# DataCanvasIO/DeepTables

Hardware: AMD Instinct MI355X
Metric: training rows/sec (fwd+bwd) DeepFM Criteo-shape batch 8192 (higher is better)
Workload: dtype f32 (split-bf16: 24-bit fwd / 16-bit bwd)

## Files before the change

### deeptables_amd/_lib.py

```python
import ctypes
import os

import torch

_HERE = os.path.dirname(os.path.abspath(__file__))
LIB_PATH = os.path.join(_HERE, 'libdt_hip.so')

_c_int = ctypes.c_int
_c_i64 = ctypes.c_int64
_c_f32 = ctypes.c_float
_ptr = ctypes.c_void_p

SIGNATURES = {
    'dt_version': (_c_int, []),
    'dt_last_error': (ctypes.c_char_p, []),
    'dt_build_arch': (ctypes.c_char_p, []),
    'dt_source_hash': (ctypes.c_char_p, []),
    'dt_graph_upload': (_c_int, [_ptr, _ptr]),
    'dt_step_trace': (_c_int, [_c_int]),
    'dt_step_trace_read': (_c_int, [_ptr, _c_int, _ptr]),
    'dt_embedding_fwd': (_c_int, [_ptr, _c_int, _ptr, _ptr, _ptr, _c_int, _c_int, _c_int, _ptr, _ptr,
                                  _ptr, _ptr]),
    'dt_embedding_bwd_dense': (_c_int, [_ptr, _ptr, _c_int, _c_int, _ptr, _ptr]),
    'dt_fm_fwd': (_c_int, [_ptr, _c_int, _c_int, _c_int, _ptr, _ptr]),
# ... 92 lines not shown
    'dt_deepfm_train_step': (_c_int, [_ptr, _c_int, _ptr, _ptr, _ptr, _ptr, _ptr, _c_int, _c_int, _c_int, _c_int,
                                      _ptr, _ptr, _ptr, _ptr, _ptr, _c_f32, _c_f32, _ptr, _ptr, _ptr, _ptr, _ptr,
                                      _ptr, _ptr, _ptr, _ptr, _ptr, _ptr, _ptr, _ptr, _ptr, _c_i64, _c_f32, _c_int, _c_int,
                                      _c_f32, _ptr, _c_f32, _ptr, _ptr]),
    'dt_deepfm_train_step_adam': (_c_int, [_ptr, _c_int, _ptr, _ptr, _ptr, _ptr, _ptr, _c_int, _c_int, _c_int, _c_int,
                                           _ptr, _ptr, _ptr, _ptr, _ptr, _c_f32, _c_f32, _ptr, _ptr, _ptr, _ptr, _ptr,
                                           _ptr, _ptr, _ptr, _ptr, _ptr, _ptr, _ptr, _ptr, _ptr, _c_i64, _c_int,
                                           _c_f32, _ptr, _c_f32, _ptr, _ptr, _ptr, _c_int, _ptr, _c_f32, _c_f32, _c_f32, _c_f32,
                                           _ptr, _ptr, _ptr, _c_i64, _c_f32, _ptr, _ptr, _ptr, _ptr]),
    'dt_deepfm_step_chains': (_c_int, [_c_int] * 5),
    'dt_deepfm_dropout_hash': (ctypes.c_uint32, [ctypes.c_uint32] * 3),
    'dt_feed_gather': (_c_int, [_ptr, _c_i64, _c_int, _ptr, _ptr, _ptr, _ptr, _ptr]),
    'dt_embedding_gather_owned': (_c_int, [_ptr, _c_int, _ptr, _ptr, _ptr, _c_int, _c_int, _c_int, _c_int, _c_int,
                                           _c_int, _ptr, _ptr, _ptr, _ptr]),
    'dt_deepfm_preelect': (_c_int, [_ptr, _c_int, _ptr, _ptr, _c_int, _c_int, _ptr, _ptr, _c_i64, _ptr]),
    'dt_deepfm_dedupe_slots': (_c_i64, [_c_int, _c_int]),
    'dt_deepfm_dedupe_bytes': (_c_i64, [_c_int, _c_int]),
    'dt_deepfm_dedupe_segments': (_c_int, [_c_int, _c_int, _ptr]),
    'dt_deepfm_dedupe_overflow_offset': (_c_i64, [_c_int, _c_int]),
    'dt_dcn_supported': (_c_int, [_c_int] * 7),
    'dt_dcn_workspace_bytes': (_c_i64, [_c_int] * 5),
    'dt_dcn_stamps_offset_floats': (_c_i64, [_c_int] * 5),
    'dt_dcn_accum_floats': (_c_i64, [_c_int] * 4),
    'dt_dcn_accum_offsets': (_c_int, [_c_int, _c_int, _c_int, _c_int, _ptr]),
    'dt_dcn_train_step': (_c_int, [_ptr, _c_int, _ptr, _ptr, _ptr, _ptr, _ptr, _c_int, _c_int, _c_int, _c_int,
                                   _ptr, _ptr, _c_int, _ptr, _ptr, _ptr, _ptr, _c_f32, _c_f32,
                                   _ptr, _ptr, _ptr, _ptr, _ptr, _ptr, _ptr,
                                   _ptr, _ptr, _ptr, _ptr, _ptr, _ptr, _ptr, _c_i64, _c_int, _c_f32, _ptr, _c_f32, _ptr, _ptr]),
    'dt_dcn_train_step_adam': (_c_int, [_ptr, _c_int, _ptr, _ptr, _ptr, _ptr, _ptr, _c_int, _c_int, _c_int, _c_int,
                                        _ptr, _ptr, _c_int, _ptr, _ptr, _ptr, _ptr, _c_f32, _c_f32,
# ... 38 lines not shown
    'dt_xdeepfm_infer_cin': (_c_int, [_c_int, _ptr, _ptr, _ptr, _c_int, _c_int, _c_int, _c_int, _c_int, _c_int, _ptr, _c_int,
                                      _c_int, _ptr, _ptr, _ptr]),
    'dt_xdeepfm_infer_head': (_c_int, [_ptr, _ptr, _c_int, _c_int, _c_int, _c_int, _c_int, _ptr, _c_int, _c_int, _ptr, _ptr,
                                       _ptr, _c_int, _ptr]),
}

DT_IDX_F32, DT_IDX_I32 = 0, 1
DT_AI_F32, DT_AI_BF16, DT_AI_BF16X2 = 0, 1, 2
DT_STEP_LOSS_MSE = 0x10
DT_STEP_SKIP_FINISH, DT_STEP_FINISH_ONLY = 0x20, 0x40
DT_STEP_TOWER_X3 = 0x80
DT_STEP_PREELECTED = 0x100
DT_STEP_TOWER_BF16 = 0x200
DT_STEP_STAMPS = 0x400
DT_STEP_PREPARED = 0x800
DT_INFER_SIGMOID, DT_INFER_TOWER_BF16 = 0x1, 0x2
DT_NET_LINEAR, DT_NET_FM, DT_NET_DNN = 0x1, 0x2, 0x4
DT_CIN_F32, DT_CIN_BF16, DT_CIN_BF16X3 = 0, 1, 2
DT_XDEEPFM_MAX_LAYERS = 8
DT_FEED_CURSOR_WORDS = 528
DT_ACT_LINEAR, DT_ACT_RELU = 0, 1
ACT_CODES = {None: 0, 'linear': 0, 'relu': 1, 'sigmoid': 2, 'tanh': 3, 'elu': 4, 'selu': 5, 'softplus': 6, 'softsign': 7,
             'exponential': 8}


def act_code(name, what):
    if name not in ACT_CODES:
        raise ValueError(f'{what} activation {name!r}: the HIP kernels fuse {sorted(k for k in ACT_CODES if k)}')
    return ACT_CODES[name]
DT_OP_KERNEL = {'mat': 0, 'vec': 1, 'num': 2}
# ... 46 lines not shown
```

### deeptables_amd/compiled.py

```python
import ctypes
import os

import torch

from . import _lib, training
from ._lib import check, lib, ptr, stream_ptr


def _hip_graph_upload(graph):
    try:
        handle = graph.raw_cuda_graph_exec()
    except (AttributeError, RuntimeError):
        return False
    return lib().dt_graph_upload(ctypes.c_void_p(int(handle)), stream_ptr()) == 0


class _old_garbage_frozen:

    def __enter__(self):
        import gc
        self.app_frozen = gc.get_freeze_count() > 0
        gc.collect()
        if not self.app_frozen:
            gc.freeze()
# ... 40 lines not shown
        self.opt_graph = None
        self._dp_steps = 0
        self._opt_graph_sig = None
        self._last_exchange_sig = None
        self._opt_graph_refused = False
        self._sig_objects = None
        self._sparse_refs = None
        self.logits = None
        self.losses = None
        self._out_refs, self._graph_out_refs, self._outputs_by_ref = {}, None, False
        self.phase_events = None
        self._first_events = None
        self._slots_per_step = False
        self.preelected = False
        self.chained = False
        self.uploaded = False
        srcs = list(feed.blocks) + ([] if self.slot_y is None else [feed.y])
        dsts = list(self.slots) + ([] if self.slot_y is None else [self.slot_y])
        nb = len(srcs)
        if nb > 8 or any((t.element_size() * (t.numel() // max(t.shape[0], 1))) % 4 for t in srcs):
            self._gather_args = False
        else:
            arr = ctypes.c_void_p * nb
            self._gather_args = (arr(*[t.data_ptr() for t in srcs]), arr(*[t.data_ptr() for t in dsts]),
                                 (ctypes.c_int * nb)(*[t.element_size() * (t.numel() // t.shape[0]) for t in srcs]), nb)

    @staticmethod
    def _nccl_backend(st):
        try:
            import torch.distributed as dist
# ... 64 lines not shown
    def steps_left(self):
        return (self.rows_available() - self.pos) // self.B

    def _gather(self, steps=None):
        n = (self.k if steps is None else steps) * self.B
        if self._gather_args is False:
            for blk, slot in zip(self.feed.blocks, self.slots):
                torch.index_select(blk, 0, self.sel[:n], out=slot[:n])
            if self.slot_y is not None:
                torch.index_select(self.feed.y, 0, self.sel[:n], out=self.slot_y[:n])
            return
        src, dst, rb, nb = self._gather_args
        check(lib().dt_feed_gather(ptr(self.order_buf), n, nb, ctypes.cast(src, ctypes.c_void_p),
                                   ctypes.cast(dst, ctypes.c_void_p), ctypes.cast(rb, ctypes.c_void_p), ptr(self.cursor),
                                   stream_ptr()), 'dt_feed_gather')

    def _step_inputs(self, i):
        s, e = i * self.B, (i + 1) * self.B
        ins = [sl[s:e] for sl in self.slots]
        yb = None if self.slot_y is None else self.slot_y[s:e]
        wb = None
        if self.feed.weighted:
            wb, yb = yb[:, -1].contiguous(), yb[:, :-1].contiguous()
            if self.feed.y_ndim == 1:
                yb = yb.reshape(-1)
        return ins, yb, wb

    def _sharded(self):
        st = self.strategy
        return self.dp and getattr(st, 'sharded_embeddings', False) and st.active and self.dm.fused_plan() is not None

    @staticmethod
    def _id_slot(i, chained):
        if not chained or i == 0:
            return i
        return 1 + ((i - 1) & 1)

    def _body(self, i, core_only=False, preelected=False, chained=False):
        dm = self.dm
        ins, yb, wb = self._step_inputs(i)
        if core_only:
            plan = dm.fused_plan()
            dm.optimizer.zero_grad(flat=False)
            loss, logit = plan.sharded_core(self.B, ins[1] if len(ins) > 1 else None, yb, self.strategy, wb)
            dm.model._dt_flat_grad = plan.accum
            return
        fused_opt = self.with_optimizer and not self.dp
        chain = {}
        if chained:
            if i + 1 < self.k:
                chain['next_ids'] = (self.slots[0][(i + 1) * self.B:(i + 2) * self.B], self._id_slot(i + 1, True))
            chain['prepared'] = i >= 1
        loss, logit = dm._forward_backward(ins, yb, wb, apply_rows=fused_opt and self.strategy is None,
                                           logit_out=None if self.logits is None else self.logits[i],
                                           slot=self._id_slot(i, chained) if self._slots_per_step else 0,
                                           preelected=preelected, **chain)
        if fused_opt:
            dm.optimizer.step()
        used_plan = getattr(dm, '_step_used_plan', False)
        if self.logits is None:
            self.logits = torch.empty((self.k,) + tuple(logit.shape), dtype=logit.dtype, device=logit.device)
            self.losses = torch.zeros(self.k, dtype=torch.float32, device=logit.device)
        self._outputs_by_ref = not used_plan and not self.dp
        if self._outputs_by_ref:
            self._out_refs[i] = (loss.detach().reshape(()), logit.detach())
        else:
            if logit.data_ptr() != self.logits[i].data_ptr():
                self.logits[i].copy_(logit)
            if not used_plan:
                self.losses[i].copy_(loss.reshape(()))
        self._losses_from_logits = bool(used_plan)

    def capture(self, warm_steps=2, collect=None):
        dm = self.dm
        dm.model.train()
        s = torch.cuda.Stream()
        s.wait_stream(torch.cuda.current_stream())
        with torch.cuda.stream(s):
            for _ in range(warm_steps):
                self._eager_steps(1, collect)
        torch.cuda.current_stream().wait_stream(s)
        torch.cuda.synchronize()
        if self._dp_graph_wanted:
            g = self._capture_dp_whole()
            if self.strategy.world_size > 1:
                import torch.distributed as dist
# ... 3 lines not shown
                    g = None
            if g is not None:
                self.graph, self.dp_graph = g, True
                import weakref
                self._owner = tuple(None if o is None else weakref.ref(o)
                                    for o in (dm.model, dm.optimizer, getattr(dm, '_fused_plan', None)))
                self.uploaded = _hip_graph_upload(g)
                torch.cuda.synchronize()
                return warm_steps
            self.k = 1
        if not self.use_graph or (self._sharded() and not self.graph_segments):
            return warm_steps
        from .models.layers import MultiColumnEmbedding
        emb_layers = [l for l in dm.model.modules() if isinstance(l, MultiColumnEmbedding)]
        core_only = self._sharded()
        plan = dm.fused_plan()
        pre = (self.k > 1 and not self.dp and not core_only and plan is not None and plan.can_preelect(self.B) and
               self.feed.kinds[0] == 'cat' and self.slots[0].dtype in (torch.int32, torch.float32))
        chain = (not pre and self.k > 1 and not self.dp and not core_only and self.with_optimizer and plan is not None and
                 plan.can_chain(self.B) and self.feed.kinds[0] == 'cat' and
                 self.slots[0].dtype in (torch.int32, torch.float32) and not self.feed.weighted)
        self.chained = bool(chain)
        self._slots_per_step = bool(pre or chain)
        self.preelected = bool(pre)
        if pre or chain:
            for i in range(1, self.k):
                plan._slot_buffers(self.B, self._id_slot(i, chain))
        g = torch.cuda.CUDAGraph()
        with _old_garbage_frozen():
            with torch.cuda.graph(g):
                if not core_only:
                    self._gather()
                if pre:
                    main = torch.cuda.current_stream()
                    side = torch.cuda.Stream()
                    side.wait_stream(main)
                    with torch.cuda.stream(side):
                        for i in range(1, self.k):
                            plan.preelect(self.slots[0][i * self.B:(i + 1) * self.B], slot=i)
                for i in range(self.k):
                    if pre and i == 1:
                        torch.cuda.current_stream().wait_stream(side)
                    self._body(i, core_only=core_only, preelected=pre and i >= 1, chained=chain)
        self._slots_per_step = False
        self._graph_out_refs = dict(self._out_refs) if self._outputs_by_ref else None
        self.graph = g
        import weakref
        self._owner = tuple(None if o is None else weakref.ref(o)
                            for o in (dm.model, dm.optimizer, getattr(dm, '_fused_plan', None)))
        self._sparse_refs = [(l, {key: list(v) for key, v in l.sparse_grads.items()}) for l in emb_layers]
        for layer in emb_layers:
            if not self.dp and self.with_optimizer:
                layer.sparse_grads.clear()
        torch.cuda.synchronize()
        self.uploaded = _hip_graph_upload(g)
        torch.cuda.synchronize()
        return warm_steps

# ... 193 lines not shown
```

### deeptables_amd/csrc/deepfm.hip

```cpp
#include <stdlib.h>
#include "tile_common.h"
#include "tower_x3.h"
#include "adam_dev.h"

namespace dt {

typedef float floatx4_t __attribute__((ext_vector_type(4)));

struct DeepFmAccum {
    int64_t dW1, dW2, db1, db2, dw3, dwo, dbo, loss, dgamma, dbeta, dwlin, slin, total;
    int64_t dw3d, dcw, dcb, sumc, sumcx;
};
__host__ __device__ inline DeepFmAccum deepfm_accum_layout(int C, int CP, int F, int Nd, int L = 0) {
    DeepFmAccum a;
    int64_t o = 0;
    a.dW1 = o; o += (int64_t)C * kH1;
    a.dW2 = o; o += (int64_t)kH1 * kH2;
    a.db1 = o; o += kH1;
    a.db2 = o; o += kH2;
    a.dw3 = o; o += (L > 0 ? C : 0);
    a.dw3d = o; o += kH2;
    a.dwo = o; o += 1;
    a.dbo = o; o += 1;
    a.loss = o; o += 2;
// ... 464 lines not shown
                }
            }
        }
    }
}
constexpr size_t kElectLds = (size_t)kElectSlots * 8 + kElectSlots / 32 * sizeof(unsigned) + 16 * sizeof(int);
constexpr size_t kElectLdsBig = kElectLds + (size_t)kElectList * sizeof(int);

__global__ __launch_bounds__(1024) void k_elect(DedupeWs dd, DeepFmDims dm, int64_t* __restrict__ rows_out) {
    extern __shared__ unsigned long long eslots_dyn[];
    ElectSync sy{nullptr, 0u};
    if (dd.seg_cur)
        elect_block_big<1024, false>(eslots_dyn, dd, dm.B, dm.F, (int)blockIdx.x, (int)threadIdx.x, rows_out, sy);
    else
        elect_block<1024, false>(eslots_dyn, dd, dm.B, dm.F, (int)blockIdx.x, (int)threadIdx.x, rows_out, sy);
}

template <int KIND>
__global__ __launch_bounds__(256) void k_rows_of_ids(const void* __restrict__ idx, const int64_t* __restrict__ row_offset,
                                                     const int32_t* __restrict__ vocab, DeepFmDims dm,
                                                     int64_t* __restrict__ rows_out, int64_t* __restrict__ rows_fm,
                                                     int* __restrict__ seg_cur, int* __restrict__ list_cur,
                                                     unsigned char* __restrict__ pid_fm, int pid_stride, int parts_log2) {
    __shared__ int64_t tile[64][129];
    if (blockIdx.x == 0 && seg_cur && (int)threadIdx.x < ((dm.F + 7) & ~7)) { seg_cur[threadIdx.x] = 0; list_cur[threadIdx.x] = 0; }
    const int b0 = blockIdx.x * 64;
    const int nb = min(64, dm.B - b0);
    for (int e = threadIdx.x; e < nb * dm.F; e += blockDim.x) {
        const int r = e / dm.F, f = e - r * dm.F;
        const int id = load_id<KIND>(idx, (int64_t)(b0 + r) * dm.F + f);
// ... 1649 lines not shown
    const DedupeLayout dl = dedupe_layout(B, F);
    const DedupeWs dd = dedupe_view(dedupe_ws, dl);
    DeepFmDims dm{B, F, 0, 0, 0, 0};
    if (idx_kind == DT_IDX_F32)
        hipLaunchKernelGGL(k_rows_of_ids<DT_IDX_F32>, dim3(ceil_div(B, 64)), dim3(256), 0, st, idx, row_offset, vocab, dm, rows_out,
                           dd.rows_fm, dd.seg_cur, dd.list_cur, dd.pid_fm, dd.pid_stride, dd.parts_log2);
    else
        hipLaunchKernelGGL(k_rows_of_ids<DT_IDX_I32>, dim3(ceil_div(B, 64)), dim3(256), 0, st, idx, row_offset, vocab, dm, rows_out,
                           dd.rows_fm, dd.seg_cur, dd.list_cur, dd.pid_fm, dd.pid_stride, dd.parts_log2);
    const size_t ldsB = dl.by_field ? kElectLdsBig : kElectLds;
    hipFuncSetAttribute((const void*)k_elect, hipFuncAttributeMaxDynamicSharedMemorySize, (int)ldsB);
    hipLaunchKernelGGL(k_elect, dim3(dl.eblocks), dim3(1024), ldsB, st, dd, dm, rows_out);
    return launch_status("dt_deepfm_preelect");
}

struct StepDense {
    float *p, *m, *v;
    int64_t n_flat;
    void* state;
    float lr;
};

struct StepChain {
    const void* next_idx;
    int64_t* next_rows_out;
    void* next_dedupe_ws;
};
static bool step_chains(const DeepFmDims& dm, int phases, bool with_dense, bool with_dedupe) {
    const bool x3_flag = (phases & (DT_STEP_TOWER_X3 | DT_STEP_TOWER_BF16)) != 0;
    return (phases & 0xf) == 2 && !(phases & (DT_STEP_SKIP_FINISH | DT_STEP_FINISH_ONLY)) && x3_flag && dm.CP <= 512 &&
// ... 85 lines not shown
    DT_REQUIRE(idx && table && row_offset && vocab && y && (dcn || w_lin) && bn_gamma && bn_beta && W1 && b1 && W2 && b2 &&
                   w3 && w_out && logit_out && rows_out && grad_rows && accum && workspace,
               "dt_deepfm_train_step: null pointer");
    DT_REQUIRE(Nd == 0 || dense, "dt_deepfm_train_step: dense is null");
    DT_REQUIRE(idx_kind == DT_IDX_F32 || idx_kind == DT_IDX_I32, "dt_deepfm_train_step: idx_kind %d", idx_kind);
    hipStream_t st = as_stream(stream);
    const DeepFmWs wl = deepfm_ws_layout(dm, Lc);
    const DeepFmAccum al = deepfm_accum_layout(dm.C, dm.CP, F, Nd, Lc);
    float* ws = reinterpret_cast<float*>(workspace);
    const int mse = (phases & DT_STEP_LOSS_MSE) ? 1 : 0;
    const bool skip_finish = (phases & DT_STEP_SKIP_FINISH) != 0, finish_only = (phases & DT_STEP_FINISH_ONLY) != 0;
    const bool bf16_flag = (phases & DT_STEP_TOWER_BF16) != 0;
    const bool x3_flag = (phases & DT_STEP_TOWER_X3) != 0 || bf16_flag;
    const bool prepared = (phases & DT_STEP_PREPARED) != 0;
    const bool preelected = (phases & DT_STEP_PREELECTED) != 0 || prepared;
    const int phases_all = phases;
    const bool stamps_flag = (phases & DT_STEP_STAMPS) != 0;
    phases &= 0xf;
    DT_REQUIRE(!(skip_finish && finish_only), "dt_deepfm_train_step: DT_STEP_SKIP_FINISH and DT_STEP_FINISH_ONLY together");
    const DcnArgs dca{cross_w, cross_b, w3, Lc, ws + wl.dXc, mse, 0, sample_weight, ws + wl.gpart, (Lc + 1) * dm.CP};
    const GPart gpt{dcn ? ws + wl.gpart : nullptr, (Lc + 1) * dm.CP, ceil_div(B, kTM), ws + wl.gsum};
    MlpParams mp{b1, W2, b2, dcn ? w3 + dm.C : w3, w_out, b_out, bn_gamma, ws + wl.mean, ws + wl.rstd, ws + wl.sc, ws + wl.betap,
                 W1, ws + wl.W1L, ws + wl.W2L, ws + wl.W2TL,
                 reinterpret_cast<const double*>(ws + wl.bnacc), bn_beta, bn_eps, bn_momentum, bn_moving_mean, bn_moving_var,
                 ws + wl.mean, ws + wl.rstd, ws + wl.sc, ws + wl.betap, ws + wl.gammap};
    DT_REQUIRE(((uintptr_t)W1 | (uintptr_t)W2 | (uintptr_t)(dcn ? W2 : w3) | (uintptr_t)accum) % 16 == 0,
               "dt_deepfm_train_step: W1 / W2 / w3 / accum must be 16-byte aligned");
    const int tiles = ceil_div(B, kTM);
    DedupeWs dd{nullptr, 0, nullptr, nullptr, nullptr, nullptr, nullptr};
    DT_REQUIRE(!(dedupe_ws && grad_rows_field_major), "dt_deepfm_train_step: dedupe and field-major row gradients "
// ... 46 lines not shown
        const int rec_blocks_f = ceil_div(part3_layout(dm.CP, Lc, 1).n, 256);
        const RecSrc rsrc_f{reinterpret_cast<const double*>(ws + wl.racc), part3_layout(dm.CP, Lc, 1).stride};
        hipLaunchKernelGGL(k_bn_grads2, dim3(dm.C + kH2 + rec_blocks_f), dim3(256), 0, st, W1, bn_gamma, bn_beta, dm,
                           accum, al, ws + wl.wpart, wgrad_row_blocks(), Lc, cross_w, cross_b, w3, rsrc_f, dm.C + kH2, gpt);
        if (drop.thr || drop.thr_dense) hipLaunchKernelGGL(k_emb_drop_advance, dim3(1), dim3(1), 0, st, dropout_seed);
        return launch_status(dcn ? "dt_dcn_train_step" : "dt_deepfm_train_step");
    }
    DT_REQUIRE(!adam || (pipe && dd.rows_fm && !grad_rows_field_major),
               "dt_deepfm_train_step_adam: the in-step row update needs a backward step with the in-step dedupe (dedupe_ws) "
               "and row-major row gradients");

    const bool chains = step_chains(dm, phases_all, adam && sdense, dd.rows_fm != nullptr);
    DT_REQUIRE(!prepared || chains, "dt_deepfm_train_step: DT_STEP_PREPARED on a step that cannot be chained (dt_deepfm_step_chains)");
    DT_REQUIRE(!(chain && chain->next_idx) || (chains && chain->next_rows_out && chain->next_dedupe_ws),
               "dt_deepfm_train_step_adam: next_idx on a step that cannot be chained, or without next_rows_out / next_dedupe_ws");
    StepNext nx{nullptr, nullptr, dd, 0};
    if (chain && chain->next_idx) {
        DT_REQUIRE((uintptr_t)chain->next_dedupe_ws % 16 == 0 && chain->next_dedupe_ws != dedupe_ws && chain->next_rows_out != rows_out,
                   "dt_deepfm_train_step_adam: the next step needs its own rows_out / dedupe_ws (16-byte aligned)");
        const DedupeLayout dln = dedupe_layout(B, F);
        nx.idx = chain->next_idx;
        nx.rows_out = chain->next_rows_out;
        nx.dd = dedupe_view(chain->next_dedupe_ws, dln);
        nx.eblocks = dln.eblocks;
    }
    const size_t ldsC = ((size_t)kTM * (dm.CP + kPad) + 4 * dm.CP + kTM * (kH1 + kPad) + kTM * kH2S + 5 * kTM +
                         (dcn ? kCrossLds + (2 * Lc + 1) * dm.CP : 0)) * sizeof(float);
    DT_UNSUPPORTED(ldsC > 160 * 1024, "dt_dcn_train_step: the tile kernel needs %zu B of LDS", ldsC);
    if (adam && sdense) {
        const int64_t want_flat = dcn ? al.dcb + (int64_t)Lc * dm.C : al.dwlin + F + Nd;
// ... 104 lines not shown
                           stamps ? stamps + (int64_t)tiles * 32 : nullptr, ep, ad, drop,                                 \
                           stamps ? stamps + (int64_t)tiles * 16 : nullptr, join_env, bnacc, (int)wl.bnacc_n, nx, gpt,    \
                           (adam && sdense) ? ws + wl.lrsnap : nullptr);                                               \
    } while (0)
        if (dcn) { if (wm == 0) DT_ED(true, 0); else if (wm == 1) DT_ED(true, 1); else DT_ED(true, 2); }
        else { if (wm == 0) DT_ED(false, 0); else if (wm == 1) DT_ED(false, 1); else DT_ED(false, 2); }
#undef DT_ED
        trace_mark(3, st);
        if (adam && sdense) {
            const int seg_blocks = 1024;
            const int small_blocks = rec_blocks;
            const DedupeLayout dl = dedupe_layout(B, F);
            const FinishSeg fs{SegTail{dd.nseg, dd.seg_row, dd.seg_off, dd.seg_cnt, dd.seg_list, dl.regions, dl.cap},
                               adam->table, adam->m, adam->v, grad_rows, adam->sstride, D};
            const DenseAdam da{sdense->p, sdense->m, sdense->v, adam->lr_t_host, adam->b1, adam->b2, adam->eps};
            const X3Lay lay = nx.idx ? X3Lay{x3_w1b, x3_w1r, x3_w2b, x3_w2r, n1, n1, n2, n2, dcn ? x3_cwp : nullptr}
                                     : X3Lay{nullptr, nullptr, nullptr, nullptr, 0, 0, 0, 0, nullptr};
            hipLaunchKernelGGL(k_finish_step, dim3(dm.C + kH2 + small_blocks + seg_blocks), dim3(256), 0, st, W1, ws + wl.gammap,
                               ws + wl.betap, dm, accum, al, ws + wl.wpart, row_blocks, da, (AdamState*)sdense->state, sdense->lr,
                               dm.C + kH2, small_blocks, seg_blocks, fs, Lc, cross_w, cross_b, w3, rsrc, lay, gpt, ws + wl.lrsnap);
            trace_mark(4, st);
        } else if (!skip_finish) {
            hipLaunchKernelGGL(k_bn_grads2, dim3(dm.C + kH2 + rec_blocks), dim3(256), 0, st, W1, bn_gamma, bn_beta, dm,
                               accum, al, ws + wl.wpart, row_blocks, Lc, cross_w, cross_b, w3, rsrc, dm.C + kH2, gpt);
        }
        if ((drop.thr || drop.thr_dense) && !skip_finish)
            hipLaunchKernelGGL(k_emb_drop_advance, dim3(1), dim3(1), 0, st, dropout_seed);
    } else {
        hipLaunchKernelGGL(k_finish_records, dim3(max(rec_blocks, 8)), dim3(256), 0, st, dm, accum, al, Lc, rsrc, bnacc,
                           (int)wl.bnacc_n);
    }
// ... 148 lines not shown
```

### deeptables_amd/fused.py

```python
import ctypes
import os

import torch

from . import _lib
from ._lib import check, lib, ptr, stream_ptr
from .ops import SparseRowGrad
from .utils import consts

def _step_loss(dm):
    ln = getattr(dm, 'loss_name', None)
    if dm.task == consts.TASK_BINARY and ln == 'binary_crossentropy':
        return 0
    if dm.task == consts.TASK_REGRESSION and ln in ('mse', 'mean_squared_error'):
        return _lib.DT_STEP_LOSS_MSE
    return None


TILE_H1, TILE_H2 = 128, 64


def _tower_widths(dnn_params):
    hu = tuple(tuple(h) for h in dnn_params.get('hidden_units', ()))
    if len(hu) != 2 or any(len(h) != 3 for h in hu):
# ... 236 lines not shown
    def can_preelect(self, B):
        st = self.dm.config.distribute_strategy
        return bool(st is None and _dedupe_in_step(self, B, True) and os.environ.get('DT_AMD_PREELECT', '0') == '1')

    def preelect(self, idx, slot):
        B = idx.shape[0]
        sb = self._slot_buffers(B, slot)
        idx = idx.contiguous()
        kind = _lib.DT_IDX_F32 if idx.dtype == torch.float32 else _lib.DT_IDX_I32
        if idx.dtype not in (torch.float32, torch.int32):
            raise ValueError('preelect: ids must be float32 or int32')
        check(lib().dt_deepfm_preelect(ptr(idx), kind, ptr(getattr(self.emb, f'row_offset_{self.key}')),
                                       ptr(getattr(self.emb, f'vocab_{self.key}')), B, self.F, ptr(sb['rows']),
                                       ptr(sb['dedupe']), sb['dedupe_slots'], stream_ptr()), 'dt_deepfm_preelect')

    def _phases(self, backward=True, part=0, pre=0, diag=True):
        phases = (2 if backward else 1) | part | _step_loss(self.dm) | pre
        if backward and part != _lib.DT_STEP_FINISH_ONLY:
            phases |= self.tower_flag | (self.diag_flag if diag else 0)
        return phases

    def _head(self, ids, kind, rows_src, dense, y, B, logit, rows, buf, oob, dedupe, dedupe_slots):
        training, bn = self.dm.model.training, self.bn
        return (ptr(ids), kind, *[ptr(t) for t in rows_src], ptr(dense), ptr(y), B, self.F, self.D, self.Nd,
                *self._net_args(), ptr(bn.gamma), ptr(bn.beta), ptr(bn.moving_mean) if training else None,
                ptr(bn.moving_variance) if training else None, float(bn.epsilon), float(bn.momentum), ptr(self.d1.kernel),
                ptr(self.d1.bias), ptr(self.d2.kernel), ptr(self.d2.bias), *self._head_weights(), ptr(self.out.bias),
                ptr(logit), ptr(rows), ptr(buf['grad_rows']), ptr(self.accum), ptr(buf['ws']), oob, dedupe, dedupe_slots)

    def _tail(self, phases, sw):
# ... 80 lines not shown
    def _whole_in_step(self, opt):
        table = self.emb.tables[self.key]
        flat = getattr(opt, '_flat', None)
        return bool(flat is not None and flat[0] is self.flat_params and flat[1] is self.accum and
                    os.environ.get('DT_AMD_STEP_IN_STEP', '1') != '0' and
                    all(id(p) in flat[5] for p in opt.params if p is not table))

    def can_chain(self, B):
        if os.environ.get('DT_AMD_CHAIN', '1') == '0' or self.dm.config.distribute_strategy is not None:
            return False
        opt = _rows_in_step(self, B, True, True) if _dedupe_in_step(self, B, True) else None
        if opt is None or not self._whole_in_step(opt):
            return False
        return bool(lib().dt_deepfm_step_chains(B, self.F, self.D, self.Nd, self._phases(diag=False)))

    def _id_buffers(self, idx, backward, dedupe, opt, slot, preelected, next_ids, prepared):
        B = idx.shape[0]
        ids = self._slot_buffers(B, slot) if (slot and dedupe) else self._buffers(B)
        pre = _lib.DT_STEP_PREELECTED if (preelected and dedupe and backward) else 0
        if preelected and not pre:
            raise _lib.DtHipError('a pre-elected step needs the in-step dedupe (backward, single process)')
        nxt = (None, None, None)
        if prepared or next_ids is not None:
            if opt is None or not dedupe:
                raise _lib.DtHipError('chained steps need the in-step dedupe and optimizer (can_chain)')
            if prepared:
                pre |= _lib.DT_STEP_PREPARED
            if next_ids is not None:
                nidx, nslot = next_ids
                if nidx.dtype != idx.dtype or nidx.shape != idx.shape or not nidx.is_contiguous() or not nslot or nslot == slot:
                    raise ValueError('next_ids: (contiguous ids like this step\'s, a slot of their own)')
                nb = self._slot_buffers(B, nslot)
                nxt = (ptr(nidx), ptr(nb['rows']), ptr(nb['dedupe']))
        return ids, pre, nxt

    def run(self, idx, dense, y, backward=True, apply_rows=False, sample_weight=None, logit_out=None, slot=0,
            preelected=False, next_ids=None, prepared=False):
        st = self.dm.config.distribute_strategy
        if self.ROW_OWNED and backward and getattr(st, 'sharded_embeddings', False) and st.active and \
                not self.emb.uses_dense_grad(self.D):
            return self._run_sharded(idx, dense, y, st, sample_weight)
        self.dm.model._dt_sharded_step = False
        B = idx.shape[0]
        buf = self._buffers(B)
        idx = idx.contiguous()
        kind = _lib.DT_IDX_F32 if idx.dtype == torch.float32 else _lib.DT_IDX_I32
        if idx.dtype not in (torch.float32, torch.int32):
            idx = idx.to(torch.int32)
        dense = None if dense is None else dense.contiguous()
        y = y.reshape(-1).contiguous()
        sw = _row_weights(sample_weight, y)
        table = self.emb.tables[self.key]
        logit = buf['logit']
        if logit_out is not None:
            if logit_out.shape != logit.shape or logit_out.dtype != logit.dtype or not logit_out.is_contiguous():
                raise ValueError(f'logit_out must be a contiguous float32 {tuple(logit.shape)} tensor')
            logit = logit_out
        dedupe = _dedupe_in_step(self, B, backward)
        opt = _rows_in_step(self, B, backward, apply_rows)
        ids, pre, nxt = self._id_buffers(idx, backward, dedupe, opt, slot, preelected, next_ids, prepared)
        head = self._head(idx, kind, (table, getattr(self.emb, f'row_offset_{self.key}'),
                                      getattr(self.emb, f'vocab_{self.key}')), dense, y, B, logit, ids['rows'], buf,
                          ptr(self.emb.oob_count) if self.emb.check_oob else None,
                          ptr(ids['dedupe']) if dedupe else None, buf['dedupe_slots'])
        if opt is not None:
            slots = opt._st(table, rows=True)
            whole = self._whole_in_step(opt)
            flat = opt._flat
            dn = (ptr(flat[0]), ptr(flat[2]), ptr(flat[3]), int(flat[4]), float(opt.lr)) if whole else (None, None, None, 0, 0.0)
            check(self._entry('train_step_adam')(
                *head, *self._tail(self._phases(pre=pre), sw), ptr(slots['m']), ptr(slots['v']), int(slots['m'].stride(0)),
                ptr(opt._state_tensor(table.device)), 0.0, opt.b1, opt.b2, opt.eps, *dn, *nxt, stream_ptr()),
                f'dt_{self.PREFIX}_train_step_adam')
            if whole:
                opt.applied_in_step()
# ... 437 lines not shown
```

### deeptables_amd/models/deepmodel.py

```python
import collections
import math
import os
import pickle
from collections import OrderedDict
from typing import Union

import numpy as np
import torch

from . import deepnets
from .layers import MultiColumnEmbedding, VarLenColumnEmbedding, dt_custom_objects
from .. import functional as F
from .. import training
from ..functional import Dense, Concatenate, Flatten, Input, Add, BatchNormalization, Dropout, Model
from ..utils import consts


def default_device():
    if not torch.cuda.is_available():
        raise RuntimeError('deeptables_amd needs a ROCm GPU (MI355X): the layers hot path has no CPU fallback.')
    return torch.device('cuda', torch.cuda.current_device())


class DeepModel:
# ... 217 lines not shown
            self._fused_plan = make_fused_plan(self)
        return self._fused_plan

    def inference_plan(self):
        from ..fused import make_inference_plan, predict_enabled
        if not predict_enabled() or self.model is None:
            return None
        if not hasattr(self, '_inference_plan'):
            self._inference_plan = make_inference_plan(self)
        return self._inference_plan

    def forward_backward(self, inputs, y, sample_weight=None, logit_out=None):
        return self._forward_backward(inputs, y, sample_weight, logit_out=logit_out)

    def _forward_backward(self, inputs, y, sample_weight=None, apply_rows=False, logit_out=None, slot=0, preelected=False,
                          next_ids=None, prepared=False):
        plan = self.fused_plan() if self.model.training else None
        if plan is not None and sample_weight is not None and not getattr(plan, 'takes_sample_weight', False):
            plan = None
        self.optimizer.zero_grad(flat=plan is None) if hasattr(self.optimizer, 'register_flat_group') \
            else self.optimizer.zero_grad()
        self._step_used_plan = plan is not None
        if plan is not None:
            cat = inputs[0]
            dense = inputs[1] if len(inputs) > 1 else None
            loss, logit = plan.run(cat, dense, y, apply_rows=apply_rows, sample_weight=sample_weight, logit_out=logit_out,
                                   slot=slot, preelected=preelected, next_ids=next_ids, prepared=prepared)
            self.model._dt_flat_grad = plan.accum
            return loss[0], logit
        self.model._dt_flat_grad = getattr(self, '_generic_flat_grad', None)
        self.model._dt_sharded_step = False
        logit = self.model(inputs)
        loss = self._loss(logit, y) if sample_weight is None else \
            training.weighted_loss(self.loss_name, logit, y, sample_weight)
        if loss.dim() == 0 and loss.dtype == torch.float32:
            loss.backward(training.unit_grad(loss.device))
        else:
            loss.backward()
        return loss.detach(), logit.detach()

    def train_step(self, inputs, y, sample_weight=None):
        strategy = self.config.distribute_strategy
# ... 341 lines not shown
```

### include/dt_hip.h

```cpp
#ifndef DT_HIP_H
#define DT_HIP_H

#include <stdint.h>

#ifdef __cplusplus
extern "C" {
#endif

#define DT_OK 0
#define DT_ERR_INVALID_ARG (-1)
#define DT_ERR_UNSUPPORTED (-2)
#define DT_ERR_LAUNCH (-3)

#define DT_IDX_F32 0
#define DT_IDX_I32 1

#define DT_ACT_LINEAR 0
#define DT_ACT_RELU 1
#define DT_ACT_SIGMOID 2
#define DT_ACT_TANH 3
#define DT_ACT_ELU 4
#define DT_ACT_SELU 5
#define DT_ACT_SOFTPLUS 6
#define DT_ACT_SOFTSIGN 7
// ... 196 lines not shown
int dt_field_pool_fwd(const float* x, int B, int F, int D, int use_max, float* z, int* argmax, void* stream);
int dt_field_pool_bwd(const float* grad_z, const int* argmax, int B, int F, int D, int use_max, float* grad_x,
                      void* stream);
int dt_field_scale_fwd(const float* x, const float* a, int B, int F, int D, float* out, void* stream);
int dt_field_scale_bwd(const float* x, const float* a, const float* grad_out, int B, int F, int D, float* grad_x,
                       float* grad_a, void* stream);

#define DT_STEP_LOSS_MSE 0x10
#define DT_STEP_SKIP_FINISH 0x20
#define DT_STEP_FINISH_ONLY 0x40
#define DT_STEP_TOWER_X3 0x80
#define DT_STEP_PREELECTED 0x100
#define DT_STEP_TOWER_BF16 0x200
#define DT_STEP_STAMPS 0x400
#define DT_STEP_PREPARED 0x800
int dt_deepfm_step_chains(int B, int F, int D, int Nd, int phases);
int dt_deepfm_preelect(const void* idx, int idx_kind, const int64_t* row_offset, const int32_t* vocab, int B, int F,
                       int64_t* rows_out, void* dedupe_ws, int64_t dedupe_slots, void* stream);
int64_t dt_deepfm_dedupe_slots(int B, int F);
int64_t dt_deepfm_dedupe_bytes(int B, int F);
int dt_deepfm_dedupe_segments(int B, int F, int64_t* out7_host);
int64_t dt_deepfm_dedupe_overflow_offset(int B, int F);
int dt_deepfm_supported(int B, int F, int D, int Nd, int H1, int H2);

int dt_dcn_supported(int B, int F, int D, int Nd, int H1, int H2, int L);
int64_t dt_dcn_workspace_bytes(int B, int F, int D, int Nd, int L);
int64_t dt_dcn_stamps_offset_floats(int B, int F, int D, int Nd, int L);
int64_t dt_dcn_accum_floats(int F, int D, int Nd, int L);
int dt_dcn_accum_offsets(int F, int D, int Nd, int L, int64_t* out12_host);
int dt_dcn_train_step(const void* idx, int idx_kind, const float* table, const int64_t* row_offset,
                      const int32_t* vocab, const float* dense, const float* y, int B, int F, int D, int Nd,
                      const float* cross_w, const float* cross_b, int L, const float* bn_gamma, const float* bn_beta,
                      float* bn_moving_mean, float* bn_moving_var, float bn_eps, float bn_momentum, const float* W1,
// ... 125 lines not shown
```

Before: 81.43 million.

## Elect deduplicated embedding rows for all chained steps in one batched launch

```diff
diff --git a/deeptables_amd/_lib.py b/deeptables_amd/_lib.py
--- a/deeptables_amd/_lib.py
+++ b/deeptables_amd/_lib.py
@@ -130,6 +130,8 @@
     'dt_embedding_gather_owned': (_c_int, [_ptr, _c_int, _ptr, _ptr, _ptr, _c_int, _c_int, _c_int, _c_int, _c_int,
                                            _c_int, _ptr, _ptr, _ptr, _ptr]),
     'dt_deepfm_preelect': (_c_int, [_ptr, _c_int, _ptr, _ptr, _c_int, _c_int, _ptr, _ptr, _c_i64, _ptr]),
+    'dt_deepfm_preelect_steps': (_c_int, [_ptr, _c_int, _ptr, _ptr, _c_int, _c_int, _c_int, _ptr, _c_i64, _ptr, _c_i64,
+                                          _c_i64, _ptr]),
     'dt_deepfm_dedupe_slots': (_c_i64, [_c_int, _c_int]),
     'dt_deepfm_dedupe_bytes': (_c_i64, [_c_int, _c_int]),
     'dt_deepfm_dedupe_segments': (_c_int, [_c_int, _c_int, _ptr]),
@@ -198,6 +200,7 @@
 DT_STEP_TOWER_BF16 = 0x200
 DT_STEP_STAMPS = 0x400
 DT_STEP_PREPARED = 0x800
+DT_STEP_NEXT_ELECTED = 0x1000
 DT_INFER_SIGMOID, DT_INFER_TOWER_BF16 = 0x1, 0x2
 DT_NET_LINEAR, DT_NET_FM, DT_NET_DNN = 0x1, 0x2, 0x4
 DT_CIN_F32, DT_CIN_BF16, DT_CIN_BF16X3 = 0, 1, 2
diff --git a/deeptables_amd/compiled.py b/deeptables_amd/compiled.py
--- a/deeptables_amd/compiled.py
+++ b/deeptables_amd/compiled.py
@@ -78,6 +78,7 @@
         self._slots_per_step = False
         self.preelected = False
         self.chained = False
+        self.elect_ahead = False
         self.uploaded = False
         srcs = list(feed.blocks) + ([] if self.slot_y is None else [feed.y])
         dsts = list(self.slots) + ([] if self.slot_y is None else [self.slot_y])
@@ -172,6 +173,12 @@
         check(lib().dt_feed_gather(ptr(self.order_buf), n, nb, ctypes.cast(src, ctypes.c_void_p),
                                    ctypes.cast(dst, ctypes.c_void_p), ctypes.cast(rb, ctypes.c_void_p), ptr(self.cursor),
                                    stream_ptr()), 'dt_feed_gather')
+        if steps is None:
+            self._elect_ahead()
+
+    def _elect_ahead(self):
+        if self.elect_ahead:
+            self.dm.fused_plan().preelect_steps(self.slots[0][:self.k * self.B], self.k)
 
     def _step_inputs(self, i):
         s, e = i * self.B, (i + 1) * self.B
@@ -188,8 +195,9 @@
         st = self.strategy
         return self.dp and getattr(st, 'sharded_embeddings', False) and st.active and self.dm.fused_plan() is not None
 
-    @staticmethod
-    def _id_slot(i, chained):
+    def _id_slot(self, i, chained):
+        if chained and self.elect_ahead:
+            return self.dm.fused_plan().ahead_slot(self.k, i)
         if not chained or i == 0:
             return i
         return 1 + ((i - 1) & 1)
@@ -206,7 +214,11 @@
         fused_opt = self.with_optimizer and not self.dp
         chain = {}
         if chained:
-            if i + 1 < self.k:
+            if self.elect_ahead:
+                if i + 1 < self.k:
+                    chain['next_elected'] = True
+                preelected = i == 0
+            elif i + 1 < self.k:
                 chain['next_ids'] = (self.slots[0][(i + 1) * self.B:(i + 2) * self.B], self._id_slot(i + 1, True))
             chain['prepared'] = i >= 1
         loss, logit = dm._forward_backward(ins, yb, wb, apply_rows=fused_opt and self.strategy is None,
@@ -228,6 +240,41 @@
             if not used_plan:
                 self.losses[i].copy_(loss.reshape(()))
         self._losses_from_logits = bool(used_plan)
+
+    def _decide_modes(self, core_only):
+        dm = self.dm
+        plan = dm.fused_plan()
+        pre = (self.k > 1 and not self.dp and not core_only and plan is not None and plan.can_preelect(self.B) and
+               self.feed.kinds[0] == 'cat' and self.slots[0].dtype in (torch.int32, torch.float32))
+        chain = (not pre and self.k > 1 and not self.dp and not core_only and self.with_optimizer and plan is not None and
+                 plan.can_chain(self.B) and self.feed.kinds[0] == 'cat' and
+                 self.slots[0].dtype in (torch.int32, torch.float32) and not self.feed.weighted)
+        self.chained = bool(chain)
+        self.elect_ahead = bool(chain and plan.elect_ahead_enabled())
+        self._slots_per_step = bool(pre or chain)
+        self.preelected = bool(pre)
+        if self.elect_ahead:
+            plan._ahead_block(self.B, self.k)
+        elif pre or chain:
+            for i in range(1, self.k):
+                plan._slot_buffers(self.B, self._id_slot(i, chain))
+        return pre, chain
+
+    def _enqueue_execution(self, core_only, pre, chain):
+        plan = self.dm.fused_plan()
+        if not core_only:
+            self._gather()
+        if pre:
+            main = torch.cuda.current_stream()
+            side = torch.cuda.Stream()
+            side.wait_stream(main)
+            with torch.cuda.stream(side):
+                for i in range(1, self.k):
+                    plan.preelect(self.slots[0][i * self.B:(i + 1) * self.B], slot=i)
+        for i in range(self.k):
+            if pre and i == 1:
+                torch.cuda.current_stream().wait_stream(side)
+            self._body(i, core_only=core_only, preelected=pre and i >= 1, chained=chain)
 
     def capture(self, warm_steps=2, collect=None):
         dm = self.dm
@@ -261,34 +308,11 @@
         from .models.layers import MultiColumnEmbedding
         emb_layers = [l for l in dm.model.modules() if isinstance(l, MultiColumnEmbedding)]
         core_only = self._sharded()
-        plan = dm.fused_plan()
-        pre = (self.k > 1 and not self.dp and not core_only and plan is not None and plan.can_preelect(self.B) and
-               self.feed.kinds[0] == 'cat' and self.slots[0].dtype in (torch.int32, torch.float32))
-        chain = (not pre and self.k > 1 and not self.dp and not core_only and self.with_optimizer and plan is not None and
-                 plan.can_chain(self.B) and self.feed.kinds[0] == 'cat' and
-                 self.slots[0].dtype in (torch.int32, torch.float32) and not self.feed.weighted)
-        self.chained = bool(chain)
-        self._slots_per_step = bool(pre or chain)
-        self.preelected = bool(pre)
-        if pre or chain:
-            for i in range(1, self.k):
-                plan._slot_buffers(self.B, self._id_slot(i, chain))
+        pre, chain = self._decide_modes(core_only)
         g = torch.cuda.CUDAGraph()
         with _old_garbage_frozen():
             with torch.cuda.graph(g):
-                if not core_only:
-                    self._gather()
-                if pre:
-                    main = torch.cuda.current_stream()
-                    side = torch.cuda.Stream()
-                    side.wait_stream(main)
-                    with torch.cuda.stream(side):
-                        for i in range(1, self.k):
-                            plan.preelect(self.slots[0][i * self.B:(i + 1) * self.B], slot=i)
-                for i in range(self.k):
-                    if pre and i == 1:
-                        torch.cuda.current_stream().wait_stream(side)
-                    self._body(i, core_only=core_only, preelected=pre and i >= 1, chained=chain)
+                self._enqueue_execution(core_only, pre, chain)
         self._slots_per_step = False
         self._graph_out_refs = dict(self._out_refs) if self._outputs_by_ref else None
         self.graph = g
diff --git a/deeptables_amd/csrc/deepfm.hip b/deeptables_amd/csrc/deepfm.hip
--- a/deeptables_amd/csrc/deepfm.hip
+++ b/deeptables_amd/csrc/deepfm.hip
@@ -502,6 +502,79 @@
         elect_block_big<1024, false>(eslots_dyn, dd, dm.B, dm.F, (int)blockIdx.x, (int)threadIdx.x, rows_out, sy);
     else
         elect_block<1024, false>(eslots_dyn, dd, dm.B, dm.F, (int)blockIdx.x, (int)threadIdx.x, rows_out, sy);
+}
+
+template <class T>
+__device__ __forceinline__ T* moved_by(T* p, int64_t bytes) { return reinterpret_cast<T*>(reinterpret_cast<char*>(p) + bytes); }
+__device__ __forceinline__ DedupeWs dedupe_at(DedupeWs dd, int64_t bytes) {
+    dd.rows_fm = moved_by(dd.rows_fm, bytes); dd.nseg = moved_by(dd.nseg, bytes); dd.seg_row = moved_by(dd.seg_row, bytes);
+    dd.seg_off = moved_by(dd.seg_off, bytes); dd.seg_cnt = moved_by(dd.seg_cnt, bytes);
+    dd.seg_list = moved_by(dd.seg_list, bytes); dd.overflow = moved_by(dd.overflow, bytes);
+    return dd;
+}
+
+template <int KIND>
+__global__ __launch_bounds__(1024) __attribute__((amdgpu_waves_per_eu(8, 8))) void k_elect_steps(const void* __restrict__ idx, const int64_t* __restrict__ row_offset,
+                                                      const int32_t* __restrict__ vocab, int B, int F, int k,
+                                                      int64_t* __restrict__ rows_out, int64_t rows_stride, DedupeWs dd0,
+                                                      int64_t dedupe_stride) {
+    extern __shared__ unsigned long long eslots_dyn[];
+    constexpr int NT = 1024, U = kElectSlots / NT;
+    unsigned long long* eslots = eslots_dyn;
+    unsigned* multi = reinterpret_cast<unsigned*>(eslots + kElectSlots);
+    int* scan = reinterpret_cast<int*>(multi + kElectSlots / 32);
+    const int j = (int)blockIdx.x >> 3;
+    const int s = 8 * (j / F) + ((int)blockIdx.x & 7), f = j % F;
+    if (s >= k) return;
+    const int tid = (int)threadIdx.x;
+    const DedupeWs dd = dedupe_at(dd0, (int64_t)s * dedupe_stride);
+    rows_out += (int64_t)s * rows_stride;
+    const int64_t id0 = (int64_t)s * B * F + f;
+    int idv[U];
+#pragma unroll
+    for (int u = 0; u < U; ++u) idv[u] = load_id<KIND>(idx, id0 + (int64_t)min(tid + NT * u, B - 1) * F);
+    const int voc = vocab[f];
+    const int64_t roff = row_offset[f];
+    const int nparts = 1 << dd.parts_log2;
+    if (f == F - 1)
+        for (int i = tid; i < ((((F + 7) >> 3) << 3) - F) << dd.parts_log2; i += NT) {
+            const int fp = F + (i >> dd.parts_log2), part = i & (nparts - 1);
+            dd.nseg[((((fp >> 3) << dd.parts_log2) | part) << 3) | (fp & 7)] = 0;
+        }
+    unsigned valid = 0u, member = 0u;
+#pragma unroll
+    for (int u = 0; u < U; ++u)
+        if (tid + NT * u < B && (unsigned)idv[u] < (unsigned)voc) valid |= 1u << u;
+    ElectSync sy{nullptr, 0u};
+    for (int part = 0; part < nparts; ++part) {
+        const int e = ((((f >> 3) << dd.parts_log2) | part) << 3) | (f & 7);
+        if (part) __syncthreads();
+        for (int i = tid; i < kElectSlots; i += NT) eslots[i] = 0ULL;
+        for (int i = tid; i < kElectSlots / 32; i += NT) multi[i] = 0u;
+        __syncthreads();
+        int myslot[U];
+#pragma unroll
+        for (int u = 0; u < U; ++u) {
+            int id = idv[u];
+            asm volatile("" : "+v"(id));
+            const int64_t row = roff + id;
+            const unsigned h = elect_hash(row);
+            myslot[u] = (((valid >> u) & 1u) && elect_part(h, dd.parts_log2) == part) ? elect_insert<false>(eslots, multi, row, h) : -1;
+        }
+        __syncthreads();
+        const int base1 = elect_segments<NT, false, false>(eslots, multi, scan, dd, B, f, e, tid, sy);
+#pragma unroll
+        for (int u = 0; u < U; ++u) {
+            if (myslot[u] < 0 || !(eslots[myslot[u]] & 0x800000ULL)) continue;
+            const unsigned long long old = atomicAdd(&eslots[myslot[u]], 1ULL);
+            dd.seg_list[base1 + (int)(old & 0x7fffffULL)] = (tid + NT * u) * F + f;
+            member |= 1u << u;
+        }
+    }
+#pragma unroll
+    for (int u = 0; u < U; ++u)
+        if (tid + NT * u < B)
+            rows_out[(int64_t)(tid + NT * u) * F + f] = (((valid & ~member) >> u) & 1u) ? roff + idv[u] : (int64_t)-1;
 }
 
 template <int KIND>
@@ -2181,6 +2254,38 @@
     return launch_status("dt_deepfm_preelect");
 }
 
+extern "C" int dt_deepfm_preelect_steps(const void* idx, int idx_kind, const int64_t* row_offset, const int32_t* vocab, int B,
+                                        int F, int k, int64_t* rows_out, int64_t rows_stride, void* dedupe_ws,
+                                        int64_t dedupe_stride, int64_t dedupe_slots, void* stream) {
+    DT_REQUIRE(idx && row_offset && vocab && rows_out && dedupe_ws && B > 0 && F > 0 && F <= 128 && k > 0,
+               "dt_deepfm_preelect_steps: bad arguments");
+    DT_REQUIRE(idx_kind == DT_IDX_F32 || idx_kind == DT_IDX_I32, "dt_deepfm_preelect_steps: idx_kind %d", idx_kind);
+    DT_REQUIRE(dedupe_slots == (int64_t)B * F, "dt_deepfm_preelect_steps: dedupe_slots=%lld must be dt_deepfm_dedupe_slots(B, F)",
+               (long long)dedupe_slots);
+    DT_UNSUPPORTED(B > kElectSlots, "dt_deepfm_preelect_steps: batches up to %d rows (B=%d): larger ones elect per step "
+                   "(dt_deepfm_preelect)", kElectSlots, B);
+    const DedupeLayout dl = dedupe_layout(B, F);
+    DT_REQUIRE((uintptr_t)dedupe_ws % 16 == 0 && dedupe_stride % 16 == 0 && (k == 1 || dedupe_stride >= dl.total),
+               "dt_deepfm_preelect_steps: dedupe_ws 16-byte aligned, dedupe_stride=%lld a multiple of 16 and at least "
+               "dt_deepfm_dedupe_bytes(B, F)", (long long)dedupe_stride);
+    DT_REQUIRE(k == 1 || rows_stride >= (int64_t)B * F, "dt_deepfm_preelect_steps: rows_stride=%lld below B * F",
+               (long long)rows_stride);
+    DT_REQUIRE(k <= (1 << 16), "dt_deepfm_preelect_steps: k=%d", k);
+    hipStream_t st = as_stream(stream);
+    const DedupeWs dd = dedupe_view(dedupe_ws, dl);
+    const int blocks = 8 * ceil_div(k, 8) * F;
+    if (idx_kind == DT_IDX_F32) {
+        hipFuncSetAttribute((const void*)k_elect_steps<DT_IDX_F32>, hipFuncAttributeMaxDynamicSharedMemorySize, (int)kElectLds);
+        hipLaunchKernelGGL(k_elect_steps<DT_IDX_F32>, dim3(blocks), dim3(1024), kElectLds, st, idx, row_offset, vocab, B, F, k,
+                           rows_out, rows_stride, dd, dedupe_stride);
+    } else {
+        hipFuncSetAttribute((const void*)k_elect_steps<DT_IDX_I32>, hipFuncAttributeMaxDynamicSharedMemorySize, (int)kElectLds);
+        hipLaunchKernelGGL(k_elect_steps<DT_IDX_I32>, dim3(blocks), dim3(1024), kElectLds, st, idx, row_offset, vocab, B, F, k,
+                           rows_out, rows_stride, dd, dedupe_stride);
+    }
+    return launch_status("dt_deepfm_preelect_steps");
+}
+
 struct StepDense {
     float *p, *m, *v;
     int64_t n_flat;
@@ -2296,6 +2401,7 @@
     const bool x3_flag = (phases & DT_STEP_TOWER_X3) != 0 || bf16_flag;
     const bool prepared = (phases & DT_STEP_PREPARED) != 0;
     const bool preelected = (phases & DT_STEP_PREELECTED) != 0 || prepared;
+    const bool next_elected = (phases & DT_STEP_NEXT_ELECTED) != 0;
     const int phases_all = phases;
     const bool stamps_flag = (phases & DT_STEP_STAMPS) != 0;
     phases &= 0xf;
@@ -2372,6 +2478,9 @@
     DT_REQUIRE(!prepared || chains, "dt_deepfm_train_step: DT_STEP_PREPARED on a step that cannot be chained (dt_deepfm_step_chains)");
     DT_REQUIRE(!(chain && chain->next_idx) || (chains && chain->next_rows_out && chain->next_dedupe_ws),
                "dt_deepfm_train_step_adam: next_idx on a step that cannot be chained, or without next_rows_out / next_dedupe_ws");
+    DT_REQUIRE(!next_elected || (chains && !(chain && chain->next_idx)),
+               "dt_deepfm_train_step_adam: DT_STEP_NEXT_ELECTED on a step that cannot be chained (dt_deepfm_step_chains), or "
+               "together with next_idx");
     StepNext nx{nullptr, nullptr, dd, 0};
     if (chain && chain->next_idx) {
         DT_REQUIRE((uintptr_t)chain->next_dedupe_ws % 16 == 0 && chain->next_dedupe_ws != dedupe_ws && chain->next_rows_out != rows_out,
@@ -2506,7 +2615,7 @@
             const FinishSeg fs{SegTail{dd.nseg, dd.seg_row, dd.seg_off, dd.seg_cnt, dd.seg_list, dl.regions, dl.cap},
                                adam->table, adam->m, adam->v, grad_rows, adam->sstride, D};
             const DenseAdam da{sdense->p, sdense->m, sdense->v, adam->lr_t_host, adam->b1, adam->b2, adam->eps};
-            const X3Lay lay = nx.idx ? X3Lay{x3_w1b, x3_w1r, x3_w2b, x3_w2r, n1, n1, n2, n2, dcn ? x3_cwp : nullptr}
+            const X3Lay lay = (nx.idx || next_elected) ? X3Lay{x3_w1b, x3_w1r, x3_w2b, x3_w2r, n1, n1, n2, n2, dcn ? x3_cwp : nullptr}
                                      : X3Lay{nullptr, nullptr, nullptr, nullptr, 0, 0, 0, 0, nullptr};
             hipLaunchKernelGGL(k_finish_step, dim3(dm.C + kH2 + small_blocks + seg_blocks), dim3(256), 0, st, W1, ws + wl.gammap,
                                ws + wl.betap, dm, accum, al, ws + wl.wpart, row_blocks, da, (AdamState*)sdense->state, sdense->lr,
diff --git a/deeptables_amd/fused.py b/deeptables_amd/fused.py
--- a/deeptables_amd/fused.py
+++ b/deeptables_amd/fused.py
@@ -274,6 +274,45 @@
                                        ptr(getattr(self.emb, f'vocab_{self.key}')), B, self.F, ptr(sb['rows']),
                                        ptr(sb['dedupe']), sb['dedupe_slots'], stream_ptr()), 'dt_deepfm_preelect')
 
+    @staticmethod
+    def elect_ahead_enabled():
+        return os.environ.get('DT_AMD_ELECT_AHEAD', '1') != '0'
+
+    @staticmethod
+    def ahead_slot(k, i):
+        return f'e{k}.{i}'
+
+    def _ahead_block(self, B, k):
+        buf = self._buffers(B)
+        blocks = buf.setdefault('ahead', {})
+        blk = blocks.get(k)
+        if blk is None:
+            n8 = (lib().dt_deepfm_dedupe_bytes(B, self.F) + 15) // 16 * 2
+            blk = {'rows': torch.empty((k, B, self.F), dtype=torch.int64, device=self.device),
+                   'dedupe': torch.zeros((k, n8), dtype=torch.int64, device=self.device)}
+            blocks[k] = blk
+            slots = buf.setdefault('slots', {})
+            for i in range(k):
+                slots[self.ahead_slot(k, i)] = {'rows': blk['rows'][i], 'dedupe': blk['dedupe'][i],
+                                                'dedupe_slots': buf['dedupe_slots']}
+        return blk
+
+    def preelect_steps(self, ids_kB, k):
+        if ids_kB.dtype not in (torch.float32, torch.int32):
+            raise ValueError('preelect_steps: ids must be float32 or int32')
+        if ids_kB.dim() != 2 or ids_kB.shape[1] != self.F or ids_kB.shape[0] % k or not ids_kB.is_contiguous():
+            raise ValueError('preelect_steps: ids [k * B, F], contiguous')
+        B = ids_kB.shape[0] // k
+        if not self.can_chain(B):
+            raise _lib.DtHipError('elections ahead of the steps need steps that can be chained (can_chain)')
+        blk = self._ahead_block(B, k)
+        kind = _lib.DT_IDX_F32 if ids_kB.dtype == torch.float32 else _lib.DT_IDX_I32
+        check(lib().dt_deepfm_preelect_steps(ptr(ids_kB), kind, ptr(getattr(self.emb, f'row_offset_{self.key}')),
+                                             ptr(getattr(self.emb, f'vocab_{self.key}')), B, self.F, k, ptr(blk['rows']),
+                                             blk['rows'].stride(0), ptr(blk['dedupe']), blk['dedupe'].stride(0) * 8,
+                                             self._buffers(B)['dedupe_slots'], stream_ptr()), 'dt_deepfm_preelect_steps')
+        return [self.ahead_slot(k, i) for i in range(k)]
+
     def _phases(self, backward=True, part=0, pre=0, diag=True):
         phases = (2 if backward else 1) | part | _step_loss(self.dm) | pre
         if backward and part != _lib.DT_STEP_FINISH_ONLY:
@@ -384,18 +423,22 @@
             return False
         return bool(lib().dt_deepfm_step_chains(B, self.F, self.D, self.Nd, self._phases(diag=False)))
 
-    def _id_buffers(self, idx, backward, dedupe, opt, slot, preelected, next_ids, prepared):
+    def _id_buffers(self, idx, backward, dedupe, opt, slot, preelected, next_ids, prepared, next_elected=False):
         B = idx.shape[0]
         ids = self._slot_buffers(B, slot) if (slot and dedupe) else self._buffers(B)
         pre = _lib.DT_STEP_PREELECTED if (preelected and dedupe and backward) else 0
         if preelected and not pre:
             raise _lib.DtHipError('a pre-elected step needs the in-step dedupe (backward, single process)')
         nxt = (None, None, None)
-        if prepared or next_ids is not None:
+        if prepared or next_ids is not None or next_elected:
             if opt is None or not dedupe:
                 raise _lib.DtHipError('chained steps need the in-step dedupe and optimizer (can_chain)')
             if prepared:
                 pre |= _lib.DT_STEP_PREPARED
+            if next_elected:
+                if next_ids is not None:
+                    raise ValueError('next_elected: the next step is elected already, next_ids would elect it again')
+                pre |= _lib.DT_STEP_NEXT_ELECTED
             if next_ids is not None:
                 nidx, nslot = next_ids
                 if nidx.dtype != idx.dtype or nidx.shape != idx.shape or not nidx.is_contiguous() or not nslot or nslot == slot:
@@ -405,7 +448,7 @@
         return ids, pre, nxt
 
     def run(self, idx, dense, y, backward=True, apply_rows=False, sample_weight=None, logit_out=None, slot=0,
-            preelected=False, next_ids=None, prepared=False):
+            preelected=False, next_ids=None, prepared=False, next_elected=False):
         st = self.dm.config.distribute_strategy
         if self.ROW_OWNED and backward and getattr(st, 'sharded_embeddings', False) and st.active and \
                 not self.emb.uses_dense_grad(self.D):
@@ -428,7 +471,7 @@
             logit = logit_out
         dedupe = _dedupe_in_step(self, B, backward)
         opt = _rows_in_step(self, B, backward, apply_rows)
-        ids, pre, nxt = self._id_buffers(idx, backward, dedupe, opt, slot, preelected, next_ids, prepared)
+        ids, pre, nxt = self._id_buffers(idx, backward, dedupe, opt, slot, preelected, next_ids, prepared, next_elected)
         head = self._head(idx, kind, (table, getattr(self.emb, f'row_offset_{self.key}'),
                                       getattr(self.emb, f'vocab_{self.key}')), dense, y, B, logit, ids['rows'], buf,
                           ptr(self.emb.oob_count) if self.emb.check_oob else None,
diff --git a/deeptables_amd/models/deepmodel.py b/deeptables_amd/models/deepmodel.py
--- a/deeptables_amd/models/deepmodel.py
+++ b/deeptables_amd/models/deepmodel.py
@@ -255,7 +255,7 @@
         return self._forward_backward(inputs, y, sample_weight, logit_out=logit_out)
 
     def _forward_backward(self, inputs, y, sample_weight=None, apply_rows=False, logit_out=None, slot=0, preelected=False,
-                          next_ids=None, prepared=False):
+                          next_ids=None, prepared=False, next_elected=False):
         plan = self.fused_plan() if self.model.training else None
         if plan is not None and sample_weight is not None and not getattr(plan, 'takes_sample_weight', False):
             plan = None
@@ -266,7 +266,8 @@
             cat = inputs[0]
             dense = inputs[1] if len(inputs) > 1 else None
             loss, logit = plan.run(cat, dense, y, apply_rows=apply_rows, sample_weight=sample_weight, logit_out=logit_out,
-                                   slot=slot, preelected=preelected, next_ids=next_ids, prepared=prepared)
+                                   slot=slot, preelected=preelected, next_ids=next_ids, prepared=prepared,
+                                   **({'next_elected': True} if next_elected else {}))
             self.model._dt_flat_grad = plan.accum
             return loss[0], logit
         self.model._dt_flat_grad = getattr(self, '_generic_flat_grad', None)
diff --git a/include/dt_hip.h b/include/dt_hip.h
--- a/include/dt_hip.h
+++ b/include/dt_hip.h
@@ -234,9 +234,13 @@
 #define DT_STEP_TOWER_BF16 0x200
 #define DT_STEP_STAMPS 0x400
 #define DT_STEP_PREPARED 0x800
+#define DT_STEP_NEXT_ELECTED 0x1000
 int dt_deepfm_step_chains(int B, int F, int D, int Nd, int phases);
 int dt_deepfm_preelect(const void* idx, int idx_kind, const int64_t* row_offset, const int32_t* vocab, int B, int F,
                        int64_t* rows_out, void* dedupe_ws, int64_t dedupe_slots, void* stream);
+int dt_deepfm_preelect_steps(const void* idx, int idx_kind, const int64_t* row_offset, const int32_t* vocab, int B, int F,
+                             int k, int64_t* rows_out, int64_t rows_stride, void* dedupe_ws, int64_t dedupe_stride,
+                             int64_t dedupe_slots, void* stream);
 int64_t dt_deepfm_dedupe_slots(int B, int F);
 int64_t dt_deepfm_dedupe_bytes(int B, int F);
 int dt_deepfm_dedupe_segments(int B, int F, int64_t* out7_host);
```

Result: no change. 81.10 million (-0.4%).
